# armlabstanford/Touch-GS

Hardware: AMD Instinct MI355X
Metric: train iters/s (whole-job views/s) + render Mpix/s, 1M Gaussians @ 1080p (higher is better)
Workload: dtype f32; 1 GPU; configs[2]: 1M Gaussians, 1080p, full Touch-GS train loop (RGB L1/SSIM + tactile depth/uncertainty loss), one view per rank per iter; gaussians=1000000, width=1920, height=1080, sh_degree=3, views=8, tiles=8160, longest_tile_list_any_view=792, max_list_hint=1022, parallelism=dp1, layout=morton (model.spatial_sort(): same scene, rows permuted), depth_loss_type=DEPTH_UNCERTAINTY_WEIGHTED_LOSS

## Files before the change

touch_gs_amd/csrc/project.hip:

```cpp
#include "tgs_adam.h"
#include "tgs_binning.h"
#include <cstddef>

namespace {

constexpr float SH_C0 = 0.28209479177387814f;
constexpr float SH_C1 = 0.4886025119029199f;
constexpr float SH_C2_0 = 1.0925484305920792f, SH_C2_1 = -1.0925484305920792f,
                SH_C2_2 = 0.31539156525252005f, SH_C2_3 = -1.0925484305920792f,
                SH_C2_4 = 0.5462742152960396f;
constexpr float SH_C3_0 = -0.5900435899266435f, SH_C3_1 = 2.890611442640554f,
                SH_C3_2 = -0.4570457994644658f, SH_C3_3 = 0.3731763325901154f,
                SH_C3_4 = -0.4570457994644658f, SH_C3_5 = 1.445305721320277f,
                SH_C3_6 = -0.5900435899266435f;
constexpr float BLUR = 0.3f;

template <int DEG>
__device__ __forceinline__ void sh_basis(float x, float y, float z, float* Y) {
  Y[0] = SH_C0;
  if constexpr (DEG >= 1) { Y[1] = -SH_C1 * y; Y[2] = SH_C1 * z; Y[3] = -SH_C1 * x; }
  if constexpr (DEG >= 2) {
    const float xx = x * x, yy = y * y, zz = z * z;
    const float xx_yy = fmaf(x, x, -yy);
    Y[4] = SH_C2_0 * x * y; Y[5] = SH_C2_1 * y * z;
// ... 392 lines not shown
  int base[TGS_GROUP];
  int hits[TGS_GROUP];
  int wave_tot[TGS_GROUP / TGS_WAVE];
  alignas(16) float seg_sum[2][16][12];
};
static_assert(offsetof(RunScan, seg_sum) % 16 == 0, "seg_sum is accessed through float4");

template <int CTRL>
__device__ __forceinline__ float row_dpp_add(float v) {
  const int s = __builtin_amdgcn_update_dpp(0, __builtin_bit_cast(int, v), CTRL, 0xf, 0xf, false);
  return v + __builtin_bit_cast(float, s);
}
__device__ __forceinline__ float row_sum16(float v) {
  v = row_dpp_add<0xB1>(v);
  v = row_dpp_add<0x4E>(v);
  v = row_dpp_add<0x141>(v);
  v = row_dpp_add<0x140>(v);
  return v;
}

__device__ __forceinline__ void group_sum_partials(const float* __restrict__ splats,
                                                   const int32_t* __restrict__ group_base,
                                                   const float* __restrict__ partials, int g, int N, float* v,
                                                   RunScan& S, int long_run) {
#pragma unroll
  for (int i = 0; i < 10; i++) v[i] = 0.f;
  const int tid = threadIdx.x;
  int hits = 0, base = 0;
  if (g < N) {
    const float4 r2 = ld4(splats + (size_t)g * TGS_SPLAT_FLOATS + 8);
    int x0, y0, w, h;
    unpack_rect(__float_as_uint(r2.z), x0, y0, w, h);
    hits = w * h;
    if (hits) base = group_base[g / TGS_GROUP] + __float_as_int(r2.w);
  }
  const bool big = hits > long_run;
  if (!__syncthreads_or(big)) {
    sum_run_serial(partials + (size_t)base * TGS_PARTIAL_FLOATS, hits, v);
    return;
  }
  const int nseg = big ? (hits + TGS_RUN_SEG - 1) / TGS_RUN_SEG : 0;
  int incl = nseg;
#pragma unroll
  for (int o = 1; o < TGS_WAVE; o <<= 1) {
    const int t = __shfl_up(incl, o);
    if ((tid & (TGS_WAVE - 1)) >= o) incl += t;
  }
  if ((tid & (TGS_WAVE - 1)) == TGS_WAVE - 1) S.wave_tot[tid / TGS_WAVE] = incl;
  S.base[tid] = base;
  S.hits[tid] = hits;
  __syncthreads();
  int my_off = incl - nseg, total = 0;
#pragma unroll
  for (int i = 0; i < TGS_GROUP / TGS_WAVE; i++) {
    if (i < tid / TGS_WAVE) my_off += S.wave_tot[i];
    total += S.wave_tot[i];
  }
  S.seg_off[tid] = my_off;
  if (tid == 0) S.seg_off[TGS_GROUP] = total;
  if (!big) sum_run_serial(partials + (size_t)base * TGS_PARTIAL_FLOATS, hits, v);
  __syncthreads();
  const int team = tid >> 4, q = tid & 15;
  for (int s0 = 0, buf = 0; s0 < total; s0 += 16, buf ^= 1) {
    const int s = s0 + team;
    if (s < total) {
      int lo = 0, hi = TGS_GROUP;
#pragma unroll
      for (int it = 0; it < 8; it++) {
        const int mid = (lo + hi) >> 1;
        if (S.seg_off[mid] <= s) lo = mid; else hi = mid;
      }
      const int k0 = (s - S.seg_off[lo]) * TGS_RUN_SEG;
      const int cnt = min(TGS_RUN_SEG, S.hits[lo] - k0);
      const float* p = partials + ((size_t)S.base[lo] + (size_t)(k0 + q)) * TGS_PARTIAL_FLOATS;
      float4 a[4], b[4];
      float2 c[4];
#pragma unroll
      for (int u = 0; u < 4; u++) {
        if (q + 16 * u < cnt) {
          a[u] = ld4_nt(p + 16 * u * TGS_PARTIAL_FLOATS);
          b[u] = ld4_nt(p + 16 * u * TGS_PARTIAL_FLOATS + 4);
          c[u] = *reinterpret_cast<const float2*>(p + 16 * u * TGS_PARTIAL_FLOATS + 8);
        }
      }
      float t[10];
#pragma unroll
      for (int i = 0; i < 10; i++) t[i] = 0.f;
#pragma unroll
      for (int u = 0; u < 4; u++) {
        if (q + 16 * u < cnt) {
          t[0] += a[u].x; t[1] += a[u].y; t[2] += a[u].z; t[3] += a[u].w;
          t[4] += b[u].x; t[5] += b[u].y; t[6] += b[u].z; t[7] += b[u].w;
          t[8] += c[u].x; t[9] += c[u].y;
        }
      }
#pragma unroll
      for (int i = 0; i < 10; i++) t[i] = row_sum16(t[i]);
      if (q == 0) {
        float* o = S.seg_sum[buf][team];
        st4(o, make_float4(t[0], t[1], t[2], t[3]));
        st4(o + 4, make_float4(t[4], t[5], t[6], t[7]));
        *reinterpret_cast<float2*>(o + 8) = make_float2(t[8], t[9]);
      }
    }
    __syncthreads();
    if (big) {
      const int e = min(my_off + nseg, s0 + 16);
      for (int sg = max(my_off, s0); sg < e; sg++) {
        const float* o = S.seg_sum[buf][sg - s0];
        const float4 x = ld4(o), y = ld4(o + 4);
        const float2 z = *reinterpret_cast<const float2*>(o + 8);
        v[0] += x.x; v[1] += x.y; v[2] += x.z; v[3] += x.w;
        v[4] += y.x; v[5] += y.y; v[6] += y.z; v[7] += y.w;
        v[8] += z.x; v[9] += z.y;
      }
    }
  }
  __syncthreads();
}

__global__ __launch_bounds__(256) void k_reduce_partials(
    CamK cam, int N, const float* __restrict__ splats, const int32_t* __restrict__ group_base,
    const float* __restrict__ partials, float* __restrict__ v_splats) {
  __shared__ RunScan S;
  const int g = blockIdx.x * 256 + threadIdx.x;
  float v[10];
  group_sum_partials(splats, group_base, partials, g, N, v, S, cam.long_run);
  if (g >= N) return;
  float* o = v_splats + (size_t)g * TGS_SPLAT_FLOATS;
  st4(o, make_float4(v[0], v[1], v[2], v[3]));
  st4(o + 4, make_float4(v[4], v[5], v[6], v[7]));
  st4(o + 8, make_float4(v[8], v[9], 0.f, 0.f));
}

__device__ __forceinline__ void geom_bwd(const CamK& cam, const float* m, const float* ls, const float* q,
                                         const float* v, float* vm, float* vls, float* vq) {
    Geom G;
    geom_eval(cam, m, ls, q, G);
    const float id = 1.0f / G.det;
    const float a = G.c11 * id, b = -G.c01 * id, c = G.c00 * id;
    const float va = v[4], vb = v[5], vc = v[6];
    const float G00 = -(a * a * va + a * b * vb + b * b * vc);
    const float G11 = -(b * b * va + b * c * vb + c * c * vc);
    const float G01 = -0.5f * (2.f * a * b * va + (a * c + b * b) * vb + 2.f * b * c * vc);
    float GT[6];
#pragma unroll
    for (int cc = 0; cc < 3; cc++) {
      GT[cc] = G00 * G.Tm[cc] + G01 * G.Tm[3 + cc];
      GT[3 + cc] = G01 * G.Tm[cc] + G11 * G.Tm[3 + cc];
    }
    float vS[9];
#pragma unroll
    for (int r = 0; r < 3; r++)
#pragma unroll
      for (int cc = 0; cc < 3; cc++) vS[3 * r + cc] = G.Tm[r] * GT[cc] + G.Tm[3 + r] * GT[3 + cc];
    const float S9[9] = {G.Sig[0], G.Sig[1], G.Sig[2], G.Sig[1], G.Sig[3], G.Sig[4],
                         G.Sig[2], G.Sig[4], G.Sig[5]};
    float vTm[6];
#pragma unroll
    for (int r = 0; r < 2; r++)
#pragma unroll
      for (int cc = 0; cc < 3; cc++)
        vTm[3 * r + cc] = 2.f * (GT[3 * r] * S9[cc] + GT[3 * r + 1] * S9[3 + cc] + GT[3 * r + 2] * S9[6 + cc]);
    const float* R = cam.R;
    const float vJ00 = vTm[0] * R[0] + vTm[1] * R[1] + vTm[2] * R[2];
    const float vJ02 = vTm[0] * R[6] + vTm[1] * R[7] + vTm[2] * R[8];
    const float vJ11 = vTm[3] * R[3] + vTm[4] * R[4] + vTm[5] * R[5];
    const float vJ12 = vTm[3] * R[6] + vTm[4] * R[7] + vTm[5] * R[8];
    const float rz = 1.0f / G.tz, rz2 = rz * rz;
    float vt[3] = {0.f, 0.f, 0.f};
    vt[2] += -(vJ00 * cam.fx + vJ11 * cam.fy) * rz2;
    if (G.inx) { vt[0] += -vJ02 * cam.fx * rz2; vt[2] += 2.f * vJ02 * cam.fx * G.tx * rz2 * rz; }
    else vt[2] += vJ02 * cam.fx * G.ucx * rz2;
    if (G.iny) { vt[1] += -vJ12 * cam.fy * rz2; vt[2] += 2.f * vJ12 * cam.fy * G.ty * rz2 * rz; }
    else vt[2] += vJ12 * cam.fy * G.ucy * rz2;
    vt[0] += v[0] * cam.fx * rz; vt[2] += -v[0] * cam.fx * G.tx * rz2;
    vt[1] += v[1] * cam.fy * rz; vt[2] += -v[1] * cam.fy * G.ty * rz2;
    vt[2] += v[2];
#pragma unroll
    for (int j = 0; j < 3; j++) vm[j] += R[j] * vt[0] + R[3 + j] * vt[1] + R[6 + j] * vt[2];
    float vR[9];
#pragma unroll
    for (int j = 0; j < 3; j++) {
      float vMj[3];
#pragma unroll
      for (int r = 0; r < 3; r++)
        vMj[r] = 2.f * (vS[3 * r] * G.Rq[j] + vS[3 * r + 1] * G.Rq[3 + j] + vS[3 * r + 2] * G.Rq[6 + j]) * G.s[j];
      const float vs = G.Rq[j] * vMj[0] + G.Rq[3 + j] * vMj[1] + G.Rq[6 + j] * vMj[2];
      vls[j] = vs * G.s[j];
      vR[j] = vMj[0] * G.s[j]; vR[3 + j] = vMj[1] * G.s[j]; vR[6 + j] = vMj[2] * G.s[j];
    }
    const float w = G.qn[0], x = G.qn[1], y = G.qn[2], z = G.qn[3];
    float vqn[4];
    vqn[0] = 2.f * (x * (vR[7] - vR[5]) + y * (vR[2] - vR[6]) + z * (vR[3] - vR[1]));
    vqn[1] = 2.f * (-2.f * x * (vR[4] + vR[8]) + y * (vR[1] + vR[3]) + z * (vR[2] + vR[6]) + w * (vR[7] - vR[5]));
    vqn[2] = 2.f * (x * (vR[1] + vR[3]) - 2.f * y * (vR[0] + vR[8]) + z * (vR[5] + vR[7]) + w * (vR[2] - vR[6]));
    vqn[3] = 2.f * (x * (vR[2] + vR[6]) + y * (vR[5] + vR[7]) - 2.f * z * (vR[0] + vR[4]) + w * (vR[3] - vR[1]));
    const float dot = w * vqn[0] + x * vqn[1] + y * vqn[2] + z * vqn[3];
    const float iq = 1.0f / G.qnorm;
#pragma unroll
    for (int j = 0; j < 4; j++) vq[j] = (vqn[j] - G.qn[j] * dot) * iq;
}

template <int DEG>
__global__ __launch_bounds__(256) void k_project_bwd(
    CamK cam, int N, const float* __restrict__ means, const float* __restrict__ log_scales,
    const float* __restrict__ quats, const float* __restrict__ opac_logit,
    const float* __restrict__ sh, int sh_stride, const float* __restrict__ splats,
    const int32_t* __restrict__ group_base, const float* __restrict__ partials,
    const float* __restrict__ v_splats, float* __restrict__ v_means,
    float* __restrict__ v_log_scales, float* __restrict__ v_quats,
    float* __restrict__ v_opac_logit, float* __restrict__ v_sh, float* __restrict__ v_color,
    float* __restrict__ v_xy, const int32_t* __restrict__ guard) {
  __shared__ RunScan S;
  const int g = blockIdx.x * 256 + threadIdx.x;
  if (guard && guard[1]) {
    if (v_color && g == 0) v_color[3 * (size_t)N + 3] = 1.f;
    return;
  }
  if (v_color && g == 0) {
    v_color[3 * (size_t)N] = cam.campos[0]; v_color[3 * (size_t)N + 1] = cam.campos[1];
    v_color[3 * (size_t)N + 2] = cam.campos[2]; v_color[3 * (size_t)N + 3] = 0.f;
  }
  float v[10];
  if (partials) group_sum_partials(splats, group_base, partials, g, N, v, S, cam.long_run);
  if (g >= N) return;
  if (!partials) {
    const float* p = v_splats + (size_t)g * TGS_SPLAT_FLOATS;
    const float4 a = ld4(p), b = ld4(p + 4);
    const float2 c = *reinterpret_cast<const float2*>(p + 8);
    v[0] = a.x; v[1] = a.y; v[2] = a.z; v[3] = a.w; v[4] = b.x; v[5] = b.y; v[6] = b.z;
    v[7] = b.w; v[8] = c.x; v[9] = c.y;
  }
  const float m[3] = {means[3 * g], means[3 * g + 1], means[3 * g + 2]};
  float vm[3] = {0.f, 0.f, 0.f};

  v_opac_logit[g] = v[3] * sigmoid_deriv(opac_logit[g]);

  if constexpr (DEG >= 0) {
    constexpr int K = (DEG + 1) * (DEG + 1);
    float dx = m[0] - cam.campos[0], dy = m[1] - cam.campos[1], dz = m[2] - cam.campos[2];
    const float inv = 1.0f / sqrtf(dx * dx + dy * dy + dz * dz);
    const float d[3] = {dx * inv, dy * inv, dz * inv};
    float Y[16];
    sh_basis<DEG>(d[0], d[1], d[2], Y);
    const float* c = sh + (size_t)g * sh_stride * 3;
    float col[3] = {0.5f, 0.5f, 0.5f};
    float ck[K][3];
#pragma unroll
    for (int k = 0; k < K; k++) {
#pragma unroll
      for (int ch = 0; ch < 3; ch++) { ck[k][ch] = c[3 * k + ch]; col[ch] += Y[k] * ck[k][ch]; }
    }
    float vr[3];
#pragma unroll
    for (int ch = 0; ch < 3; ch++) vr[ch] = (col[ch] > 0.f) ? v[7 + ch] : 0.f;
    if (v_color) { v_color[3 * g] = vr[0]; v_color[3 * g + 1] = vr[1]; v_color[3 * g + 2] = vr[2]; }
    if (v_sh) {
      float* o_sh = v_sh + (size_t)g * sh_stride * 3;
#pragma unroll
      for (int k = 0; k < K; k++) {
        o_sh[3 * k] = Y[k] * vr[0]; o_sh[3 * k + 1] = Y[k] * vr[1]; o_sh[3 * k + 2] = Y[k] * vr[2];
      }
      for (int k = K; k < sh_stride; k++) { o_sh[3 * k] = 0.f; o_sh[3 * k + 1] = 0.f; o_sh[3 * k + 2] = 0.f; }
    }
    if constexpr (DEG >= 1) {
      float dY[K][3];
      sh_basis_grad<DEG>(d[0], d[1], d[2], dY);
      float vd[3] = {0.f, 0.f, 0.f};
#pragma unroll
      for (int k = 1; k < K; k++) {
        const float s = ck[k][0] * vr[0] + ck[k][1] * vr[1] + ck[k][2] * vr[2];
        vd[0] += dY[k][0] * s; vd[1] += dY[k][1] * s; vd[2] += dY[k][2] * s;
      }
      const float dot = d[0] * vd[0] + d[1] * vd[1] + d[2] * vd[2];
#pragma unroll
      for (int j = 0; j < 3; j++) vm[j] += (vd[j] - d[j] * dot) * inv;
    }
  } else {
    if (v_sh) {
      float* o_sh = v_sh + (size_t)g * sh_stride * 3;
      for (int k = 0; k < sh_stride * 3; k++) o_sh[k] = 0.f;
    }
    if (v_color) { v_color[3 * g] = 0.f; v_color[3 * g + 1] = 0.f; v_color[3 * g + 2] = 0.f; }
  }

  float vls[3] = {0.f, 0.f, 0.f};
  float vq[4] = {0.f, 0.f, 0.f, 0.f};
  const bool visible = splats[(size_t)g * TGS_SPLAT_FLOATS + 4] > 0.f;
  if (visible) {
    const float ls[3] = {log_scales[3 * g], log_scales[3 * g + 1], log_scales[3 * g + 2]};
    const float4 q4 = ld4(quats + 4 * (size_t)g);
    const float q[4] = {q4.x, q4.y, q4.z, q4.w};
    geom_bwd(cam, m, ls, q, v, vm, vls, vq);
  }
  v_means[3 * g] = vm[0]; v_means[3 * g + 1] = vm[1]; v_means[3 * g + 2] = vm[2];
  v_log_scales[3 * g] = vls[0]; v_log_scales[3 * g + 1] = vls[1]; v_log_scales[3 * g + 2] = vls[2];
  st4(v_quats + 4 * (size_t)g, make_float4(vq[0], vq[1], vq[2], vq[3]));
  if (v_xy) {
    v_xy[2 * g] = v[0]; v_xy[2 * g + 1] = v[1];
  }
}

template <int DEG, int KS, bool FUSE_ADAM, bool COLOR_ONLY = false>
__global__ __launch_bounds__(256) void k_project_bwd_lds(
    CamK cam, int N, float* __restrict__ means, float* __restrict__ log_scales,
    float* __restrict__ quats, float* __restrict__ opac_logit, float* __restrict__ sh,
    const float* __restrict__ splats, const int32_t* __restrict__ group_base,
    const float* __restrict__ partials, float* __restrict__ v_means,
    float* __restrict__ v_log_scales, float* __restrict__ v_quats,
    float* __restrict__ v_opac_logit, float* __restrict__ v_sh, float* __restrict__ v_xy,
    AdamK ad_in, float* __restrict__ exp_avg, float* __restrict__ exp_avg_sq, NextView nx) {
  if (ad_in.guard && ad_in.guard[1]) {
    if (COLOR_ONLY && blockIdx.x == 0 && threadIdx.x == 0) v_sh[3 * (size_t)N + 3] = 1.f;
    return;
  }
  const AdamK ad = FUSE_ADAM ? adam_resolve(ad_in) : ad_in;
  constexpr int K = (DEG + 1) * (DEG + 1);
  static_assert(KS >= K && (3 * KS) % 4 == 0, "storage must hold the active degree in whole float4s");
  static_assert(256 * (3 * KS + 4) * sizeof(float) >= sizeof(GroupScan), "the group scan of the front prefetch reuses the SH image");
  constexpr int ROW = 3 * KS, RS = ROW + 4, F4 = ROW / 4;
  extern __shared__ float4 lds4[];
  float* lds = reinterpret_cast<float*>(lds4);
  const int tid = threadIdx.x;
  const int g0 = blockIdx.x * 256;
  const int g = g0 + tid;
  const int nrows = min(256, N - g0);
  const size_t blk = (size_t)g0 * ROW;

  static_assert(256 * (3 * KS + 4) * sizeof(float) >= sizeof(RunScan), "the run scan reuses the SH image");
  float v[10];
  group_sum_partials(splats, group_base, partials, g, N, v, *reinterpret_cast<RunScan*>(lds4), cam.long_run);
  {
    const int nf = nrows * F4;
    for (int f0 = tid; f0 < nf; f0 += 256 * 4) {
      float4 t[4];
#pragma unroll
      for (int u = 0; u < 4; u++)
        if (f0 + 256 * u < nf) {
          const float* src = sh + blk + 4 * (size_t)(f0 + 256 * u);
          t[u] = FUSE_ADAM ? ld4(src) : ld4_nt(src);
        }
#pragma unroll
      for (int u = 0; u < 4; u++) {
        const int f = f0 + 256 * u;
        if (f < nf) { const int row = f / F4, c4 = f - row * F4; st4(lds + row * RS + 4 * c4, t[u]); }
      }
    }
  }
  __syncthreads();

  float vm[3] = {0.f, 0.f, 0.f}, vls[3] = {0.f, 0.f, 0.f}, vq[4] = {0.f, 0.f, 0.f, 0.f};
  float m[3] = {0.f, 0.f, 0.f}, ls[3] = {0.f, 0.f, 0.f}, q[4] = {1.f, 0.f, 0.f, 0.f};
  float ol = 0.f, vol = 0.f;
  if constexpr (COLOR_ONLY) {
    if (g == 0) {
      v_sh[3 * (size_t)N] = cam.campos[0]; v_sh[3 * (size_t)N + 1] = cam.campos[1];
      v_sh[3 * (size_t)N + 2] = cam.campos[2]; v_sh[3 * (size_t)N + 3] = 0.f;
    }
  }
  if (g < N) {
    m[0] = means[3 * g]; m[1] = means[3 * g + 1]; m[2] = means[3 * g + 2];
    ol = opac_logit[g];
    vol = v[3] * sigmoid_deriv(ol);
    float dx = m[0] - cam.campos[0], dy = m[1] - cam.campos[1], dz = m[2] - cam.campos[2];
    const float inv = 1.0f / sqrtf(dx * dx + dy * dy + dz * dz);
    const float d[3] = {dx * inv, dy * inv, dz * inv};
    float Y[16];
    sh_basis<DEG>(d[0], d[1], d[2], Y);
    float* row = lds + tid * RS;
    float ck[ROW];
#pragma unroll
    for (int i = 0; i < F4; i++) {
      const float4 t = ld4(row + 4 * i);
      ck[4 * i] = t.x; ck[4 * i + 1] = t.y; ck[4 * i + 2] = t.z; ck[4 * i + 3] = t.w;
    }
    float col[3] = {0.5f, 0.5f, 0.5f};
#pragma unroll
    for (int k = 0; k < K; k++)
#pragma unroll
      for (int ch = 0; ch < 3; ch++) col[ch] += Y[k] * ck[3 * k + ch];
    float vr[3];
#pragma unroll
    for (int ch = 0; ch < 3; ch++) vr[ch] = (col[ch] > 0.f) ? v[7 + ch] : 0.f;
    if constexpr (DEG >= 1) {
      float dY[K][3];
      sh_basis_grad<DEG>(d[0], d[1], d[2], dY);
      float vd[3] = {0.f, 0.f, 0.f};
#pragma unroll
      for (int k = 1; k < K; k++) {
        const float s = ck[3 * k] * vr[0] + ck[3 * k + 1] * vr[1] + ck[3 * k + 2] * vr[2];
        vd[0] += dY[k][0] * s; vd[1] += dY[k][1] * s; vd[2] += dY[k][2] * s;
      }
      const float dot = d[0] * vd[0] + d[1] * vd[1] + d[2] * vd[2];
#pragma unroll
      for (int j = 0; j < 3; j++) vm[j] += (vd[j] - d[j] * dot) * inv;
    }
    if constexpr (COLOR_ONLY) { v_sh[3 * g] = vr[0]; v_sh[3 * g + 1] = vr[1]; v_sh[3 * g + 2] = vr[2]; }
#pragma unroll
    for (int i = 0; i < (COLOR_ONLY ? 0 : F4); i++) {
      float4 t;
      t.x = (4 * i) / 3 < K ? Y[(4 * i) / 3] * vr[(4 * i) % 3] : 0.f;
      t.y = (4 * i + 1) / 3 < K ? Y[(4 * i + 1) / 3] * vr[(4 * i + 1) % 3] : 0.f;
      t.z = (4 * i + 2) / 3 < K ? Y[(4 * i + 2) / 3] * vr[(4 * i + 2) % 3] : 0.f;
      t.w = (4 * i + 3) / 3 < K ? Y[(4 * i + 3) / 3] * vr[(4 * i + 3) % 3] : 0.f;
      st4(row + 4 * i, t);
    }
    if (splats[(size_t)g * TGS_SPLAT_FLOATS + 4] > 0.f) {
      ls[0] = log_scales[3 * g]; ls[1] = log_scales[3 * g + 1]; ls[2] = log_scales[3 * g + 2];
      const float4 q4 = ld4(quats + 4 * (size_t)g);
      q[0] = q4.x; q[1] = q4.y; q[2] = q4.z; q[3] = q4.w;
      geom_bwd(cam, m, ls, q, v, vm, vls, vq);
    } else if (FUSE_ADAM) {
      ls[0] = log_scales[3 * g]; ls[1] = log_scales[3 * g + 1]; ls[2] = log_scales[3 * g + 2];
      const float4 q4 = ld4(quats + 4 * (size_t)g);
      q[0] = q4.x; q[1] = q4.y; q[2] = q4.z; q[3] = q4.w;
    }
    if (v_xy) { v_xy[2 * g] = v[0]; v_xy[2 * g + 1] = v[1]; }
    if constexpr (!FUSE_ADAM) {
      v_means[3 * g] = vm[0]; v_means[3 * g + 1] = vm[1]; v_means[3 * g + 2] = vm[2];
      v_log_scales[3 * g] = vls[0]; v_log_scales[3 * g + 1] = vls[1]; v_log_scales[3 * g + 2] = vls[2];
      st4(v_quats + 4 * (size_t)g, make_float4(vq[0], vq[1], vq[2], vq[3]));
      v_opac_logit[g] = vol;
    } else {
      float* ea = exp_avg; float* es = exp_avg_sq;
#pragma unroll
      for (int j = 0; j < 3; j++) {
        const long long e = 3ll * g + j;
        float pm = m[j], M = ea[e], V = es[e];
        adam1(ad, ad.lr_means, pm, vm[j], M, V);
        means[3 * g + j] = pm; ea[e] = M; es[e] = V;
        m[j] = pm;
      }
#pragma unroll
      for (int j = 0; j < 3; j++) {
        const long long e = ad.e_means + 3ll * g + j;
        float pl = ls[j], M = ea[e], V = es[e];
        adam1(ad, ad.lr_scales, pl, vls[j], M, V);
        log_scales[3 * g + j] = pl; ea[e] = M; es[e] = V;
        ls[j] = pl;
      }
      {
        const long long e = ad.e_scales + 4ll * g;
        float4 M = ld4_nt(ea + e), V = ld4_nt(es + e);
        float4 Q = make_float4(q[0], q[1], q[2], q[3]);
        adam1(ad, ad.lr_quats, Q.x, vq[0], M.x, V.x); adam1(ad, ad.lr_quats, Q.y, vq[1], M.y, V.y);
        adam1(ad, ad.lr_quats, Q.z, vq[2], M.z, V.z); adam1(ad, ad.lr_quats, Q.w, vq[3], M.w, V.w);
        st4_nt(quats + 4 * (size_t)g, Q); st4_nt(ea + e, M); st4_nt(es + e, V);
        q[0] = Q.x; q[1] = Q.y; q[2] = Q.z; q[3] = Q.w;
      }
      {
        const long long e = ad.e_quats + g;
        float po = ol, M = ea[e], V = es[e];
        adam1(ad, ad.lr_opac, po, vol, M, V);
        opac_logit[g] = po; ea[e] = M; es[e] = V;
        ol = po;
      }
    }
  }
  if constexpr (COLOR_ONLY) return;
  __syncthreads();
  const int nf = nrows * F4;
  for (int f0 = tid; f0 < nf; f0 += 256 * 2) {
    if constexpr (!FUSE_ADAM) {
#pragma unroll
      for (int u = 0; u < 2; u++) {
        const int f = f0 + 256 * u;
        if (f < nf) { const int row = f / F4, c4 = f - row * F4; st4(v_sh + blk + 4 * (size_t)f, ld4(lds + row * RS + 4 * c4)); }
      }
    } else {
      float4 P[2], M[2], V[2];
#pragma unroll
      for (int u = 0; u < 2; u++) {
        const int f = f0 + 256 * u;
        if (f < nf) {
          const size_t e = blk + 4 * (size_t)f;
          P[u] = ld4_nt(sh + e); M[u] = ld4_nt(exp_avg + ad.e_opac + e); V[u] = ld4_nt(exp_avg_sq + ad.e_opac + e);
        }
      }
#pragma unroll
      for (int u = 0; u < 2; u++) {
        const int f = f0 + 256 * u;
        if (f < nf) {
          const int row = f / F4, c4 = f - row * F4;
          const float4 G = ld4(lds + row * RS + 4 * c4);
          const size_t e = blk + 4 * (size_t)f;
          const int c = 4 * c4;
          adam1(ad, c < 3 ? ad.lr_dc : ad.lr_rest, P[u].x, G.x, M[u].x, V[u].x);
          adam1(ad, c + 1 < 3 ? ad.lr_dc : ad.lr_rest, P[u].y, G.y, M[u].y, V[u].y);
          adam1(ad, c + 2 < 3 ? ad.lr_dc : ad.lr_rest, P[u].z, G.z, M[u].z, V[u].z);
          adam1(ad, ad.lr_rest, P[u].w, G.w, M[u].w, V[u].w);
          st4_nt(sh + e, P[u]); st4_nt(exp_avg + ad.e_opac + e, M[u]); st4_nt(exp_avg_sq + ad.e_opac + e, V[u]);
          if (nx.colors) st4(lds + row * RS + 4 * c4, P[u]);
        }
      }
    }
  }
  if constexpr (FUSE_ADAM) {
    if (nx.colors) {
      __syncthreads();
      float rgb[3] = {0.f, 0.f, 0.f};
      if (g < N) {
        sh_color<DEG>(m, nx.campos, lds + tid * RS, rgb);
        nx.colors[3 * g] = rgb[0]; nx.colors[3 * g + 1] = rgb[1]; nx.colors[3 * g + 2] = rgb[2];
      }
      if (nx.fr.splats) {
        __syncthreads();
        project_fwd_core<true>(nx.fr.cam, N, g, m, ls, q, ol, rgb, nx.fr.splats, nx.fr.radii, nx.fr.group_base,
                               nx.fr.tile_count, nx.fr.rank, nx.fr.status, nx.fr.capacity, nx.fr.sticky,
                               reinterpret_cast<GroupScan*>(lds4));
      }
      if (g == 0) *nx.tag = nx.tag_value;
    }
  }
}

template <int DEG>
__global__ __launch_bounds__(256) void k_adam_sh_gathered(
    int world, int row0, int N, int sh_stride, const float* __restrict__ means,
    float* __restrict__ sh, const float* __restrict__ v_color_all, AdamK ad_in,
    float* __restrict__ exp_avg, float* __restrict__ exp_avg_sq) {
  if (ad_in.guard && ad_in.guard[1]) return;
  const AdamK ad = adam_resolve(ad_in);
  constexpr int K = (DEG + 1) * (DEG + 1);
  const int ROW = 3 * sh_stride, RS = ROW + 4, F4 = ROW / 4;
  extern __shared__ float4 lds4[];
  float* lds = reinterpret_cast<float*>(lds4);
  const int tid = threadIdx.x;
  const int g0 = row0 + blockIdx.x * 256;
  const int g = g0 + tid;
  const int nrows = min(256, N - g0);
  const size_t blk = (size_t)g0 * ROW;
  if (g < N) {
    const float m0 = means[3 * g], m1 = means[3 * g + 1], m2 = means[3 * g + 2];
    float acc[3 * K];
#pragma unroll
    for (int i = 0; i < 3 * K; i++) acc[i] = 0.f;
    const size_t nb = (size_t)(N - row0);
    const size_t blk_r = 3 * nb + 4;
    for (int r = 0; r < world; r++) {
      const float* vc = v_color_all + r * blk_r + 3 * (size_t)(g - row0);
      const float* cp = v_color_all + r * blk_r + 3 * nb;
      const float v0 = vc[0], v1 = vc[1], v2 = vc[2];
      const float dx = m0 - cp[0], dy = m1 - cp[1], dz = m2 - cp[2];
      const float inv = 1.0f / sqrtf(dx * dx + dy * dy + dz * dz);
      float Y[16];
      sh_basis<DEG>(dx * inv, dy * inv, dz * inv, Y);
#pragma unroll
      for (int k = 0; k < K; k++) {
        acc[3 * k] = fmaf(Y[k], v0, acc[3 * k]);
        acc[3 * k + 1] = fmaf(Y[k], v1, acc[3 * k + 1]);
        acc[3 * k + 2] = fmaf(Y[k], v2, acc[3 * k + 2]);
      }
    }
    float* row = lds + tid * RS;
#pragma unroll
    for (int i = 0; i < 3 * K / 4; i++) st4(row + 4 * i, make_float4(acc[4 * i], acc[4 * i + 1], acc[4 * i + 2], acc[4 * i + 3]));
    if constexpr ((3 * K) % 4 != 0) {
      float t[4] = {0.f, 0.f, 0.f, 0.f};
#pragma unroll
      for (int i = 0; i < (3 * K) % 4; i++) t[i] = acc[(3 * K / 4) * 4 + i];
      st4(row + (3 * K / 4) * 4, make_float4(t[0], t[1], t[2], t[3]));
    }
    for (int i = (3 * K + 3) / 4; i < F4; i++) st4(row + 4 * i, make_float4(0.f, 0.f, 0.f, 0.f));
  }
  __syncthreads();
  const int nf = nrows * F4;
  for (int f0 = tid; f0 < nf; f0 += 256 * 2) {
    float4 P[2], M[2], V[2];
#pragma unroll
    for (int u = 0; u < 2; u++) {
      const int f = f0 + 256 * u;
      if (f < nf) {
        const size_t e = blk + 4 * (size_t)f;
        P[u] = ld4_nt(sh + e); M[u] = ld4_nt(exp_avg + ad.e_opac + e); V[u] = ld4_nt(exp_avg_sq + ad.e_opac + e);
      }
    }
#pragma unroll
    for (int u = 0; u < 2; u++) {
      const int f = f0 + 256 * u;
      if (f < nf) {
        const int row = f / F4, c4 = f - row * F4;
        const float4 G = ld4(lds + row * RS + 4 * c4);
        const size_t e = blk + 4 * (size_t)f;
        const int c = 4 * c4;
        adam1(ad, c < 3 ? ad.lr_dc : ad.lr_rest, P[u].x, G.x, M[u].x, V[u].x);
        adam1(ad, c + 1 < 3 ? ad.lr_dc : ad.lr_rest, P[u].y, G.y, M[u].y, V[u].y);
        adam1(ad, c + 2 < 3 ? ad.lr_dc : ad.lr_rest, P[u].z, G.z, M[u].z, V[u].z);
        adam1(ad, ad.lr_rest, P[u].w, G.w, M[u].w, V[u].w);
        st4_nt(sh + e, P[u]); st4_nt(exp_avg + ad.e_opac + e, M[u]); st4_nt(exp_avg_sq + ad.e_opac + e, V[u]);
      }
    }
  }
}

struct ChunkTable {
  int n;
  int begin[9];
  const float* blk[8];
};

template <int DEG>
__global__ __launch_bounds__(256) void k_adam_sh_geom_next(
    CamK cam, int world, int N, int sh_stride, float* __restrict__ means, float* __restrict__ log_scales,
    float* __restrict__ quats, float* __restrict__ opac_logit, float* __restrict__ sh, const float* __restrict__ grads,
    ChunkTable ct, AdamK ad_in, float* __restrict__ exp_avg, float* __restrict__ exp_avg_sq,
    float* __restrict__ splats, int32_t* __restrict__ radii, int32_t* __restrict__ group_base,
    int32_t* __restrict__ tile_count, int32_t* __restrict__ rank, int32_t* __restrict__ status,
    long long capacity, int32_t* __restrict__ sticky, int32_t* __restrict__ tag, int32_t tag_value) {
  if (ad_in.guard && ad_in.guard[1]) return;
  const AdamK ad = adam_resolve(ad_in);
  constexpr int K = (DEG + 1) * (DEG + 1);
  const int ROW = 3 * sh_stride, RS = ROW + 4, F4 = ROW / 4;
  extern __shared__ float4 lds4[];
  float* lds = reinterpret_cast<float*>(lds4);
  const int tid = threadIdx.x;
  const int g0 = blockIdx.x * 256;
  const int g = g0 + tid;
  const int nrows = min(256, N - g0);
  const size_t blk = (size_t)g0 * ROW;
  int row0 = 0, rows_c = N;
  const float* v_color_all = ct.blk[0];
#pragma unroll
  for (int c = 0; c < 8; c++)
    if (c < ct.n && g0 >= ct.begin[c] && g0 < ct.begin[c + 1]) { row0 = ct.begin[c]; rows_c = ct.begin[c + 1] - ct.begin[c]; v_color_all = ct.blk[c]; }
  float m[3] = {0.f, 0.f, 0.f}, ls[3] = {0.f, 0.f, 0.f}, q[4] = {1.f, 0.f, 0.f, 0.f}, rgb[3] = {0.f, 0.f, 0.f};
  float ol = 0.f;
  if (g < N) {
    m[0] = means[3 * g]; m[1] = means[3 * g + 1]; m[2] = means[3 * g + 2];
    float acc[3 * K];
#pragma unroll
    for (int i = 0; i < 3 * K; i++) acc[i] = 0.f;
    const size_t nb = (size_t)rows_c;
    const size_t blk_r = 3 * nb + 4;
    for (int r = 0; r < world; r++) {
      const float* vc = v_color_all + r * blk_r + 3 * (size_t)(g - row0);
      const float* cp = v_color_all + r * blk_r + 3 * nb;
      const float v0 = vc[0], v1 = vc[1], v2 = vc[2];
      const float dx = m[0] - cp[0], dy = m[1] - cp[1], dz = m[2] - cp[2];
      const float inv = 1.0f / sqrtf(dx * dx + dy * dy + dz * dz);
      float Y[16];
      sh_basis<DEG>(dx * inv, dy * inv, dz * inv, Y);
#pragma unroll
      for (int k = 0; k < K; k++) {
        acc[3 * k] = fmaf(Y[k], v0, acc[3 * k]);
        acc[3 * k + 1] = fmaf(Y[k], v1, acc[3 * k + 1]);
        acc[3 * k + 2] = fmaf(Y[k], v2, acc[3 * k + 2]);
      }
    }
    float* row = lds + tid * RS;
#pragma unroll
    for (int i = 0; i < 3 * K / 4; i++) st4(row + 4 * i, make_float4(acc[4 * i], acc[4 * i + 1], acc[4 * i + 2], acc[4 * i + 3]));
    if constexpr ((3 * K) % 4 != 0) {
      float t[4] = {0.f, 0.f, 0.f, 0.f};
#pragma unroll
      for (int i = 0; i < (3 * K) % 4; i++) t[i] = acc[(3 * K / 4) * 4 + i];
      st4(row + (3 * K / 4) * 4, make_float4(t[0], t[1], t[2], t[3]));
    }
    for (int i = (3 * K + 3) / 4; i < F4; i++) st4(row + 4 * i, make_float4(0.f, 0.f, 0.f, 0.f));
  }
  __syncthreads();
  const int nf = nrows * F4;
  for (int f0 = tid; f0 < nf; f0 += 256 * 2) {
    float4 P[2], M[2], V[2];
#pragma unroll
    for (int u = 0; u < 2; u++) {
      const int f = f0 + 256 * u;
      if (f < nf) {
        const size_t e = blk + 4 * (size_t)f;
        P[u] = ld4_nt(sh + e); M[u] = ld4_nt(exp_avg + ad.e_opac + e); V[u] = ld4_nt(exp_avg_sq + ad.e_opac + e);
      }
    }
#pragma unroll
    for (int u = 0; u < 2; u++) {
      const int f = f0 + 256 * u;
      if (f < nf) {
        const int row = f / F4, c4 = f - row * F4;
        const float4 G = ld4(lds + row * RS + 4 * c4);
        const size_t e = blk + 4 * (size_t)f;
        const int c = 4 * c4;
        adam1(ad, c < 3 ? ad.lr_dc : ad.lr_rest, P[u].x, G.x, M[u].x, V[u].x);
        adam1(ad, c + 1 < 3 ? ad.lr_dc : ad.lr_rest, P[u].y, G.y, M[u].y, V[u].y);
        adam1(ad, c + 2 < 3 ? ad.lr_dc : ad.lr_rest, P[u].z, G.z, M[u].z, V[u].z);
        adam1(ad, ad.lr_rest, P[u].w, G.w, M[u].w, V[u].w);
        st4_nt(sh + e, P[u]); st4_nt(exp_avg + ad.e_opac + e, M[u]); st4_nt(exp_avg_sq + ad.e_opac + e, V[u]);
        st4(lds + row * RS + 4 * c4, P[u]);
      }
    }
  }
  __syncthreads();
  if (g < N) {
#pragma unroll
    for (int j = 0; j < 3; j++) {
      const long long e = 3ll * g + j;
      float P = m[j], M = exp_avg[e], V = exp_avg_sq[e];
      adam1(ad, ad.lr_means, P, grads[e], M, V);
      means[3 * g + j] = P; exp_avg[e] = M; exp_avg_sq[e] = V;
      m[j] = P;
    }
#pragma unroll
    for (int j = 0; j < 3; j++) {
      const long long e = ad.e_means + 3ll * g + j;
      float P = log_scales[3 * g + j], M = exp_avg[e], V = exp_avg_sq[e];
      adam1(ad, ad.lr_scales, P, grads[e], M, V);
      log_scales[3 * g + j] = P; exp_avg[e] = M; exp_avg_sq[e] = V;
      ls[j] = P;
    }
    {
      const long long e = ad.e_scales + 4ll * g;
      float4 Q = ld4(quats + 4 * (size_t)g), G = ld4_nt(grads + e), M = ld4_nt(exp_avg + e), V = ld4_nt(exp_avg_sq + e);
      adam1(ad, ad.lr_quats, Q.x, G.x, M.x, V.x); adam1(ad, ad.lr_quats, Q.y, G.y, M.y, V.y);
      adam1(ad, ad.lr_quats, Q.z, G.z, M.z, V.z); adam1(ad, ad.lr_quats, Q.w, G.w, M.w, V.w);
      st4(quats + 4 * (size_t)g, Q); st4_nt(exp_avg + e, M); st4_nt(exp_avg_sq + e, V);
      q[0] = Q.x; q[1] = Q.y; q[2] = Q.z; q[3] = Q.w;
    }
    {
      const long long e = ad.e_quats + g;
      float P = opac_logit[g], M = exp_avg[e], V = exp_avg_sq[e];
      adam1(ad, ad.lr_opac, P, grads[e], M, V);
      opac_logit[g] = P; exp_avg[e] = M; exp_avg_sq[e] = V;
      ol = P;
    }
    sh_color<DEG>(m, cam.campos, lds + tid * RS, rgb);
  }
  __syncthreads();
  project_fwd_core<true>(cam, N, g, m, ls, q, ol, rgb, splats, radii, group_base, tile_count, rank, status,
                         capacity, sticky, reinterpret_cast<GroupScan*>(lds4));
  if (g == 0) *tag = tag_value;
}

template <int DEG, bool BWD>
__global__ __launch_bounds__(256) void k_sh_op(int N, int sh_stride, const float* __restrict__ dirs,
                                               const float* __restrict__ coeffs_or_vout,
                                               float* __restrict__ out) {
  constexpr int K = (DEG + 1) * (DEG + 1);
  const int g = blockIdx.x * 256 + threadIdx.x;
  if (g >= N) return;
  float dx = dirs[3 * g], dy = dirs[3 * g + 1], dz = dirs[3 * g + 2];
  const float inv = 1.0f / sqrtf(dx * dx + dy * dy + dz * dz);
  float Y[16];
  sh_basis<DEG>(dx * inv, dy * inv, dz * inv, Y);
  if constexpr (!BWD) {
    const float* c = coeffs_or_vout + (size_t)g * sh_stride * 3;
    float r = 0.f, gg = 0.f, b = 0.f;
#pragma unroll
    for (int k = 0; k < K; k++) { r += Y[k] * c[3 * k]; gg += Y[k] * c[3 * k + 1]; b += Y[k] * c[3 * k + 2]; }
    out[3 * g] = r; out[3 * g + 1] = gg; out[3 * g + 2] = b;
  } else {
    const float v0 = coeffs_or_vout[3 * g], v1 = coeffs_or_vout[3 * g + 1], v2 = coeffs_or_vout[3 * g + 2];
    float* o = out + (size_t)g * sh_stride * 3;
#pragma unroll
    for (int k = 0; k < K; k++) { o[3 * k] = Y[k] * v0; o[3 * k + 1] = Y[k] * v1; o[3 * k + 2] = Y[k] * v2; }
    for (int k = K; k < sh_stride; k++) { o[3 * k] = 0.f; o[3 * k + 1] = 0.f; o[3 * k + 2] = 0.f; }
  }
}

inline bool lds_k8_ok(int sh_deg, int sh_stride) {
  return (sh_stride == 16 && sh_deg >= 0 && sh_deg <= 3) || (sh_stride == 4 && sh_deg >= 0 && sh_deg <= 1);
}
#define DISPATCH_DEG_KS(M, deg, ks)                                                              \
  do {                                                                                           \
    if ((ks) == 16) {                                                                            \
      switch (deg) { case 0: M(0, 16); break; case 1: M(1, 16); break; case 2: M(2, 16); break;  \
                     default: M(3, 16); break; }                                                 \
    } else {                                                                                     \
      if ((deg) == 0) M(0, 4); else M(1, 4);                                                     \
    }                                                                                            \
  } while (0)

}

extern "C" int tgs_project_fwd(const TgsCamera* cam, int N, const float* means,
                               const float* log_scales, const float* quats,
                               const float* opac_logit, const float* sh, int sh_stride, int sh_deg,
                               const float* colors_in, float* splats, int32_t* radii,
                               void* stream) {
  TGS_CHECK_ARG(camera_ok(cam), "bad camera");
  TGS_CHECK_ARG(N >= 0, "N < 0");
  TGS_CHECK_ARG(cam->W <= 4080 && cam->H <= 4080, "image side > 4080 px (255 tiles)");
  if (N == 0) return TGS_OK;
  TGS_CHECK_ARG(means && log_scales && quats && opac_logit && splats, "null pointer");
  if (!sh) sh_deg = -1;
  TGS_CHECK_ARG(sh_deg <= 3, "sh_deg > 3");
  TGS_CHECK_ARG(sh_deg < 0 || sh_stride >= (sh_deg + 1) * (sh_deg + 1), "sh_stride too small");
  const CamK k = make_camk(cam);
  const dim3 grid((N + 255) / 256), block(256);
  hipStream_t s = (hipStream_t)stream;
#define LAUNCH(D)                                                                              \
  hipLaunchKernelGGL((k_project_fwd<D, false>), grid, block, 0, s, k, N, means, log_scales, quats, \
                     opac_logit, sh, sh_stride, colors_in, splats, radii, (int32_t*)nullptr,       \
                     (int32_t*)nullptr, (int32_t*)nullptr, (int32_t*)nullptr, 0ll, (int32_t*)nullptr)
  switch (sh_deg) {
    case 0: LAUNCH(0); break;
    case 1: LAUNCH(1); break;
    case 2: LAUNCH(2); break;
    case 3: LAUNCH(3); break;
    default: LAUNCH(-1); break;
  }
#undef LAUNCH
  TGS_CHECK_LAUNCH();
  return TGS_OK;
}

// ... 543 lines not shown
```

Measured before the change: 1017 iters/s.

## Recompute SH gradients in the fused Adam sweep instead of staging and rereading SH

In the fused-Adam backward, each thread no longer writes its full per-row SH gradient into shared memory. It stores only (vr, inv) in the row's padding slot. The Adam sweep then recomputes the SH basis from the means and rebuilds each float4 of gradient on the fly. The SH parameters staged in shared memory are reused as P, so the second global read of sh is gone, and the means/scales/quats/opacity Adam update moves after the SH sweep. This cuts HBM traffic on the SH coefficients at the cost of extra ALU work (recomputed SH basis per float4) and an added read of means per element.

```diff
diff --git a/touch_gs_amd/csrc/project.hip b/touch_gs_amd/csrc/project.hip
--- a/touch_gs_amd/csrc/project.hip
+++ b/touch_gs_amd/csrc/project.hip
@@ -718,6 +718,37 @@
   }
 }
 
+
+template <int DEG, int KS>
+__device__ __forceinline__ float4 sh_grad4(const float* Y, float4 w, int c4) {
+  constexpr int K = (DEG + 1) * (DEG + 1);
+  static_assert(KS % 4 == 0, "a row is a whole number of basis quads");
+  const int a = c4 / 3, b = c4 - 3 * a;
+  float q[4];
+#pragma unroll
+  for (int t = 0; t < 4; t++) q[t] = t < K ? Y[t] : 0.f;
+#pragma unroll
+  for (int i = 1; 4 * i < K; i++)
+    if (a == i) {
+#pragma unroll
+      for (int t = 0; t < 4; t++) q[t] = 4 * i + t < K ? Y[4 * i + t] : 0.f;
+    }
+  const float y0 = b == 0 ? q[0] : b == 1 ? q[1] : q[2];
+  const float y1 = b == 0 ? q[0] : b == 1 ? q[1] : q[3];
+  const float y2 = b == 0 ? q[0] : b == 1 ? q[2] : q[3];
+  const float y3 = b == 0 ? q[1] : b == 1 ? q[2] : q[3];
+  const float v0 = b == 0 ? w.x : b == 1 ? w.y : w.z;
+  const float v1 = b == 0 ? w.y : b == 1 ? w.z : w.x;
+  const float v2 = b == 0 ? w.z : b == 1 ? w.x : w.y;
+  const int k0 = 4 * a + b, k1 = 4 * a + (b == 2 ? 3 : b), k2 = 4 * a + (b == 0 ? 0 : b + 1), k3 = 4 * a + b + 1;
+  float4 G;
+  G.x = (K == KS || k0 < K) ? y0 * v0 : 0.f;
+  G.y = (K == KS || k1 < K) ? y1 * v1 : 0.f;
+  G.z = (K == KS || k2 < K) ? y2 * v2 : 0.f;
+  G.w = (K == KS || k3 < K) ? y3 * v0 : 0.f;
+  return G;
+}
+
 template <int DEG, int KS, bool FUSE_ADAM, bool COLOR_ONLY = false>
 __global__ __launch_bounds__(256) void k_project_bwd_lds(
     CamK cam, int N, float* __restrict__ means, float* __restrict__ log_scales,
@@ -754,8 +785,7 @@
 #pragma unroll
       for (int u = 0; u < 4; u++)
         if (f0 + 256 * u < nf) {
-          const float* src = sh + blk + 4 * (size_t)(f0 + 256 * u);
-          t[u] = FUSE_ADAM ? ld4(src) : ld4_nt(src);
+          t[u] = ld4_nt(sh + blk + 4 * (size_t)(f0 + 256 * u));
         }
 #pragma unroll
       for (int u = 0; u < 4; u++) {
@@ -813,8 +843,9 @@
       for (int j = 0; j < 3; j++) vm[j] += (vd[j] - d[j] * dot) * inv;
     }
     if constexpr (COLOR_ONLY) { v_sh[3 * g] = vr[0]; v_sh[3 * g + 1] = vr[1]; v_sh[3 * g + 2] = vr[2]; }
-#pragma unroll
-    for (int i = 0; i < (COLOR_ONLY ? 0 : F4); i++) {
+    if constexpr (FUSE_ADAM) st4(row + ROW, make_float4(vr[0], vr[1], vr[2], inv));
+#pragma unroll
+    for (int i = 0; i < (COLOR_ONLY || FUSE_ADAM ? 0 : F4); i++) {
       float4 t;
       t.x = (4 * i) / 3 < K ? Y[(4 * i) / 3] * vr[(4 * i) % 3] : 0.f;
       t.y = (4 * i + 1) / 3 < K ? Y[(4 * i + 1) / 3] * vr[(4 * i + 1) % 3] : 0.f;
@@ -838,7 +869,64 @@
       v_log_scales[3 * g] = vls[0]; v_log_scales[3 * g + 1] = vls[1]; v_log_scales[3 * g + 2] = vls[2];
       st4(v_quats + 4 * (size_t)g, make_float4(vq[0], vq[1], vq[2], vq[3]));
       v_opac_logit[g] = vol;
+    }
+  }
+  if constexpr (COLOR_ONLY) return;
+  __syncthreads();
+  const int nf = nrows * F4;
+  for (int f0 = tid; f0 < nf; f0 += 256 * 2) {
+    if constexpr (!FUSE_ADAM) {
+#pragma unroll
+      for (int u = 0; u < 2; u++) {
+        const int f = f0 + 256 * u;
+        if (f < nf) { const int row = f / F4, c4 = f - row * F4; st4(v_sh + blk + 4 * (size_t)f, ld4(lds + row * RS + 4 * c4)); }
+      }
     } else {
+      float4 M[2], V[2];
+      float mr[2][3];
+#pragma unroll
+      for (int u = 0; u < 2; u++) {
+        const int f = f0 + 256 * u;
+        if (f < nf) {
+          const size_t e = blk + 4 * (size_t)f;
+          M[u] = ld4_nt(exp_avg + ad.e_opac + e); V[u] = ld4_nt(exp_avg_sq + ad.e_opac + e);
+          if constexpr (DEG >= 1) {
+            const float* mp = means + 3 * (size_t)(g0 + f / F4);
+            mr[u][0] = mp[0]; mr[u][1] = mp[1]; mr[u][2] = mp[2];
+          }
+        }
+      }
+#pragma unroll
+      for (int u = 0; u < 2; u++) {
+        const int f = f0 + 256 * u;
+        if (f < nf) {
+          const int row = f / F4, c4 = f - row * F4;
+          float4 P = ld4(lds + row * RS + 4 * c4);
+          const float4 w = ld4(lds + row * RS + ROW);
+          float Y[16];
+          if constexpr (DEG >= 1) {
+            float dx = mr[u][0] - cam.campos[0], dy = mr[u][1] - cam.campos[1], dz = mr[u][2] - cam.campos[2];
+            const float d[3] = {dx * w.w, dy * w.w, dz * w.w};
+            sh_basis<DEG>(d[0], d[1], d[2], Y);
+          } else {
+            sh_basis<DEG>(0.f, 0.f, 0.f, Y);
+          }
+          const float4 G = sh_grad4<DEG, KS>(Y, w, c4);
+          const size_t e = blk + 4 * (size_t)f;
+          const int c = 4 * c4;
+          adam1(ad, c < 3 ? ad.lr_dc : ad.lr_rest, P.x, G.x, M[u].x, V[u].x);
+          adam1(ad, c + 1 < 3 ? ad.lr_dc : ad.lr_rest, P.y, G.y, M[u].y, V[u].y);
+          adam1(ad, c + 2 < 3 ? ad.lr_dc : ad.lr_rest, P.z, G.z, M[u].z, V[u].z);
+          adam1(ad, ad.lr_rest, P.w, G.w, M[u].w, V[u].w);
+          st4_nt(sh + e, P); st4_nt(exp_avg + ad.e_opac + e, M[u]); st4_nt(exp_avg_sq + ad.e_opac + e, V[u]);
+          if (nx.colors) st4(lds + row * RS + 4 * c4, P);
+        }
+      }
+    }
+  }
+  if constexpr (FUSE_ADAM) {
+    __syncthreads();
+    if (g < N) {
       float* ea = exp_avg; float* es = exp_avg_sq;
 #pragma unroll
       for (int j = 0; j < 3; j++) {
@@ -873,48 +961,7 @@
         ol = po;
       }
     }
-  }
-  if constexpr (COLOR_ONLY) return;
-  __syncthreads();
-  const int nf = nrows * F4;
-  for (int f0 = tid; f0 < nf; f0 += 256 * 2) {
-    if constexpr (!FUSE_ADAM) {
-#pragma unroll
-      for (int u = 0; u < 2; u++) {
-        const int f = f0 + 256 * u;
-        if (f < nf) { const int row = f / F4, c4 = f - row * F4; st4(v_sh + blk + 4 * (size_t)f, ld4(lds + row * RS + 4 * c4)); }
-      }
-    } else {
-      float4 P[2], M[2], V[2];
-#pragma unroll
-      for (int u = 0; u < 2; u++) {
-        const int f = f0 + 256 * u;
-        if (f < nf) {
-          const size_t e = blk + 4 * (size_t)f;
-          P[u] = ld4_nt(sh + e); M[u] = ld4_nt(exp_avg + ad.e_opac + e); V[u] = ld4_nt(exp_avg_sq + ad.e_opac + e);
-        }
-      }
-#pragma unroll
-      for (int u = 0; u < 2; u++) {
-        const int f = f0 + 256 * u;
-        if (f < nf) {
-          const int row = f / F4, c4 = f - row * F4;
-          const float4 G = ld4(lds + row * RS + 4 * c4);
-          const size_t e = blk + 4 * (size_t)f;
-          const int c = 4 * c4;
-          adam1(ad, c < 3 ? ad.lr_dc : ad.lr_rest, P[u].x, G.x, M[u].x, V[u].x);
-          adam1(ad, c + 1 < 3 ? ad.lr_dc : ad.lr_rest, P[u].y, G.y, M[u].y, V[u].y);
-          adam1(ad, c + 2 < 3 ? ad.lr_dc : ad.lr_rest, P[u].z, G.z, M[u].z, V[u].z);
-          adam1(ad, ad.lr_rest, P[u].w, G.w, M[u].w, V[u].w);
-          st4_nt(sh + e, P[u]); st4_nt(exp_avg + ad.e_opac + e, M[u]); st4_nt(exp_avg_sq + ad.e_opac + e, V[u]);
-          if (nx.colors) st4(lds + row * RS + 4 * c4, P[u]);
-        }
-      }
-    }
-  }
-  if constexpr (FUSE_ADAM) {
     if (nx.colors) {
-      __syncthreads();
       float rgb[3] = {0.f, 0.f, 0.f};
       if (g < N) {
         sh_color<DEG>(m, nx.campos, lds + tid * RS, rgb);
```

Measured after the change: 1016 iters/s. About the same (-0.2%).
